# RishWijewardhena/vision-textile-inspection

Hardware: AMD Instinct MI355X
Metric: frames/sec whole-node, YOLOv8n-seg 640x640 bs=64; mask IoU vs CPU ref (higher is better)
Workload: dtype f16x2

## Files before the change

### vision-textile-inspection_amd/csrc/conv.hip

```cpp
#include <algorithm>
#include <cstdlib>
#include <type_traits>

#include "conv_dev.h"

namespace vti {

__host__ __device__ inline int patch_dim(int t, int ks, int s, int mode) { return mode == 1 ? t : (t - 1) * s + ks; }

size_t stem_lds_bytes(int TH, int TW);

bool conv_wreg_ok(int ks, int stride, int mode, int WN, int NREP, int threads) {
    return mode == 0 && ks == 1 && stride == 1 && threads == 256 && WN == 4 && NREP <= 4;
}

size_t conv_lds_bytes(int ks, int stride, int mode, int TH, int TW, int WN, int NREP, int wreg) {
    if (mode == 1) return stem_lds_bytes(TH, TW);
    const int npix = patch_dim(TH, ks, stride, mode) * patch_dim(TW, ks, stride, mode);
    const size_t plane = (size_t)((npix + 15) & ~15) * 16;
    const int taps = mode == 1 ? 1 : ks * ks;
    size_t raw = 0;
    if (mode == 1) raw = (((size_t)(2 * TH + 1) * (2 * TW + 1) * 3) + 15) & ~(size_t)15;
    return 4 * plane + (wreg ? 0 : (size_t)WN * NREP * taps * 1024) + raw;
}

template <typename T, int KS, int S, int NREP, int WN, int NREP2 = 0, int NT = 256, bool WREG = false>
__global__ __launch_bounds__(NT, NT == 512 ? 1 : 2) void conv_kernel(const ConvParams p) {
    using vec = typename Tr<T>::vec;
    constexpr int VEC = Tr<T>::VEC, KC = Tr<T>::KC;
    constexpr int TAPS = KS * KS, PAD = KS / 2;
    constexpr int NTB = WN * NREP;
    constexpr int PP = NT / 4;
    constexpr int AR = NT == 512 ? 6 : (S == 2 ? 12 : 8);
    constexpr int BR = (NTB * TAPS * 64 + NT - 1) / NT;
    static_assert(!WREG || (KS == 1 && WN == NT / 64 && NREP2 == 0 && BR == NREP && NREP < 5), "WREG: one consumer wave per fragment");
    constexpr unsigned OOB = 0xFFFFFFFFu;
    extern __shared__ __attribute__((aligned(16))) char smem[];

    const int tid = threadIdx.x, lane = tid & 63, wave = tid >> 6;
    const int wn = wave % WN, wm = wave / WN;
    int t = blockIdx.x;
    const int tx = t % p.tiles_x; t /= p.tiles_x;
    const int ty = t % p.tiles_y;
    const int b = t / p.tiles_y;
    const int oy0 = ty * p.TH, ox0 = tx * p.TW;
    const int PH = (p.TH - 1) * S + KS, PW = (p.TW - 1) * S + KS;
    const int npix = PH * PW;
    const int plane_bytes = ((npix + 15) & ~15) * 16;
    char* smA = smem;
    char* smB = smem + 4 * plane_bytes;
    const int nt0 = blockIdx.y * NTB;
    const int tile_px = p.TH * p.TW;
    VTI_STAMP(0);

    int abase[MREP], opy[MREP], opx[MREP];
    bool pvalid[MREP];
#pragma unroll
    for (int m = 0; m < MREP; ++m) {
        const int pp = (wm * MREP + m) * 16 + (lane & 15);
        const bool v = pp < tile_px;
        const int pc = v ? pp : 0;
        const int py = (int)__umulhi((unsigned)pc, p.tw_magic), px = pc - py * p.TW;
        opy[m] = oy0 + py; opx[m] = ox0 + px;
        pvalid[m] = v && opy[m] < p.Hout && opx[m] < p.Wout;
        abase[m] = (lane >> 4) * plane_bytes + ((py * S) * PW + px * S) * 16;
    }

    f32x4 acc[MREP][NREP];
#pragma unroll
    for (int m = 0; m < MREP; ++m)
#pragma unroll
        for (int n = 0; n < NREP; ++n) acc[m][n] = (f32x4){0.f, 0.f, 0.f, 0.f};

    const size_t frame_elems = (size_t)p.Hin * p.Win * p.in_ld;
    const __amdgpu_buffer_rsrc_t rsA = __builtin_amdgcn_make_buffer_rsrc(
        (void*)((const T*)p.in + (size_t)b * frame_elems), 0, (int)(frame_elems * sizeof(T)), 0x00020000);
    const __amdgpu_buffer_rsrc_t rsB = __builtin_amdgcn_make_buffer_rsrc((void*)p.wpk, 0, (int)p.wpk_bytes, 0x00020000);

    const int iy0 = oy0 * S - PAD, ix0 = ox0 * S - PAD;
    const int q = (tid >> 3) & 3;
    const int pix0 = (tid >> 5) * 8 + (tid & 7);
    const int ldsA0 = q * plane_bytes + pix0 * 16;
    const int cvalid = (p.Cin - q * VEC + KC - 1) / KC;
    unsigned aoff[AR];
#pragma unroll
    for (int u = 0; u < AR; ++u) {
        const int pix = pix0 + PP * u;
        const int py = (int)__umulhi((unsigned)pix, p.pw_magic), px = pix - py * PW;
        const int y = iy0 + py, x = ix0 + px;
        const bool ok = pix < npix && (unsigned)y < (unsigned)p.Hin && (unsigned)x < (unsigned)p.Win;
        aoff[u] = ok ? (unsigned)(((y * p.Win + x) * p.in_ld + p.in_coff + q * VEC) * (int)sizeof(T)) : OOB;
    }
    constexpr bool BPRE = NREP < 5 || NT == 512;
    constexpr int PD = (KS == 1 && BPRE) ? 2 : 1;
    vec ra[PD][AR], rb[PD][BR];
    auto loadB = [&](int c, vec (&rbs)[BR]) {
        const unsigned sB = (unsigned)(((size_t)c * p.ntiles_n + nt0) * (TAPS * 1024));
#pragma unroll
        for (int u = 0; u < BR; ++u) {
            if constexpr (WREG) rbs[u] = buf_load16<vec>(rsB, (unsigned)((wn * NREP + u) * 64 + lane) * 16u, sB);
            else if (tid + u * NT < NTB * TAPS * 64) rbs[u] = buf_load16<vec>(rsB, (unsigned)(tid + u * NT) * 16u, sB);
        }
    };
    auto issue = [&](int c, vec (&ras)[AR], vec (&rbs)[BR]) {
        const bool qok = c < cvalid;
#pragma unroll
        for (int u = 0; u < AR; ++u)
            if (pix0 + PP * u < ((npix + 7) & ~7))
                ras[u] = buf_load16<vec>(rsA, qok ? aoff[u] : OOB, (unsigned)(c * KC * (int)sizeof(T)));
        if constexpr (BPRE) loadB(c, rbs);
    };
    auto commit = [&](int c, vec (&ras)[AR], vec (&rbs)[BR]) {
        if constexpr (!BPRE) loadB(c, rbs);
#pragma unroll
        for (int u = 0; u < AR; ++u)
            if (pix0 + PP * u < npix) *(vec*)(smA + ldsA0 + u * (PP * 16)) = ras[u];
        if constexpr (!WREG) {
#pragma unroll
            for (int u = 0; u < BR; ++u)
                if (tid + u * NT < NTB * TAPS * 64) *(vec*)(smB + (tid + u * NT) * 16) = rbs[u];
        }
    };
    auto chunk = [&](int c, auto set_c) {
        constexpr int SET = decltype(set_c)::value;
        if (c < 2) VTI_STAMP(1 + 5 * c);
        commit(c, ra[SET], rb[SET]);
        if (c < 2) VTI_STAMP(3 + 5 * c);
        __syncthreads();
        if (c < 2) VTI_STAMP(4 + 5 * c);
        constexpr int WD = NREP >= 5 ? 1 : 2;
        vec wq[WD][NREP];
        if constexpr (WREG) {
#pragma unroll
            for (int n = 0; n < NREP; ++n) wq[0][n] = rb[SET][n];
        }
        if (c + PD < p.nchunks) issue(c + PD, ra[SET], rb[SET]);
        {
            constexpr int NSTEP = TAPS * MREP;
            constexpr int XD = NREP >= 5 ? 2 : 3;
            vec xq[XD];
            auto ldx = [&](int s_) -> vec {
                const int tp = s_ / MREP, mm = s_ % MREP;
                const int toff = ((tp / KS) * PW + (tp % KS)) * 16;
                return *(const vec*)(smA + abase[mm] + toff);
            };
            auto ldw = [&](int tp, vec (&w)[NREP]) {
#pragma unroll
                for (int n = 0; n < NREP; ++n)
                    w[n] = *(const vec*)(smB + ((wn * NREP + n) * TAPS + tp) * 1024 + lane * 16);
            };
            if constexpr (Tr<T>::H2 && TAPS > 1 && (NREP <= 3 || (NREP == 4 && NT == 512))) {
                auto ldw1 = [&](int tp, int n) -> vec { return *(const vec*)(smB + ((wn * NREP + n) * TAPS + tp) * 1024 + lane * 16); };
                h2_taps<NREP, MREP, TAPS, 3>(acc, ldx, ldw1);
            } else {
            if constexpr (!WREG) ldw(0, wq[0]);
            xq[0] = ldx(0);
            if (XD > 2 && NSTEP > 1) xq[1] = ldx(1);
#pragma unroll
            for (int s_ = 0; s_ < NSTEP; ++s_) {
                const int tp = s_ / MREP, mm = s_ % MREP;
                if (s_ + XD - 1 < NSTEP) xq[(s_ + XD - 1) % XD] = ldx(s_ + XD - 1);
                if (WD == 2 && mm == 0 && tp + 1 < TAPS) ldw(tp + 1, wq[(tp + 1) % WD]);
                __builtin_amdgcn_sched_barrier(0);
#pragma unroll
                for (int n = 0; n < NREP; ++n) acc[mm][n] = mma(wq[tp % WD][n], xq[s_ % XD], acc[mm][n]);
                __builtin_amdgcn_sched_barrier(0);
                if (WD == 1 && mm == MREP - 1 && tp + 1 < TAPS) ldw(tp + 1, wq[0]);
            }
            }
        }
        if (c < 2) VTI_STAMP(5 + 5 * c);
        if (c + 1 < p.nchunks) __syncthreads();
    };

    issue(0, ra[0], rb[0]);
    if constexpr (PD == 2) {
        if (p.nchunks > 1) issue(1, ra[1], rb[1]);
        for (int c = 0; c < p.nchunks; c += 2) {
            chunk(c, std::integral_constant<int, 0>{});
            if (c + 1 < p.nchunks) chunk(c + 1, std::integral_constant<int, 1>{});
        }
    } else {
        for (int c = 0; c < p.nchunks; ++c) chunk(c, std::integral_constant<int, 0>{});
    }

    VTI_STAMP(11);
    if constexpr (NREP2 == 0) {
        conv_epilogue<T, NREP>(p, acc, pvalid, opy, opx, b, nt0, wn, lane);
    } else {
        static_assert(WN == 1, "fused stage needs the whole Cout in one wave");
        conv_stage2<T, NREP, NREP2>(p, acc, pvalid, opy, opx, b, lane);
    }
    VTI_STAMP(12);
}

size_t convfold_lds_bytes(int TH, int TW) {
    const int npix = (TH + 2) * (TW + 2);
    return 4 * (size_t)((npix + 15) & ~15) * 16 + (size_t)16 * 4 * 1024;
}
bool convfold_supported(int c_in, int c_mid, int c_out, int ntiles2) {
    return c_in == c_mid && c_mid % 16 == 0 && c_out == 64 && c_in % 16 == 0 && c_in <= 64 && combo_has(FoldN2{}, ntiles2);
}

template <typename T, int NREP2, int NT = 256>
__global__ __launch_bounds__(NT, NT == 512 ? 1 : 2) void convfold_kernel(const ConvParams p) {
    using vec = typename Tr<T>::vec;
    constexpr int VEC = Tr<T>::VEC, KC = Tr<T>::KC;
    constexpr int NREP = 4, TAPS = 4, NTB = 16, AR = 8;
    constexpr int BR = NTB * TAPS * 64 / NT;
    constexpr int PPP = NT / 4;
    constexpr unsigned OOB = 0xFFFFFFFFu;
    extern __shared__ __attribute__((aligned(16))) char smem[];

    const int tid = threadIdx.x, lane = tid & 63, wave = (tid >> 6) & 3, mgrp = tid >> 8;
    const int py = wave >> 1, px = wave & 1;
    int t = blockIdx.x;
    const int tx = t % p.tiles_x; t /= p.tiles_x;
    const int ty = t % p.tiles_y;
    const int b = t / p.tiles_y;
    const int oy0 = ty * p.TH, ox0 = tx * p.TW;
    const int PH = p.TH + 2, PW = p.TW + 2;
    const int npix = PH * PW;
    const int plane_bytes = ((npix + 15) & ~15) * 16;
    char* smA = smem;
    char* smB = smem + 4 * plane_bytes;
    const int tile_px = p.TH * p.TW;

    int abase[MREP], opy[MREP], opx[MREP];
    bool pvalid[MREP];
#pragma unroll
    for (int m = 0; m < MREP; ++m) {
        const int pp = (mgrp * MREP + m) * 16 + (lane & 15);
        const bool v = pp < tile_px;
        const int pc = v ? pp : 0;
        const int ly = (int)__umulhi((unsigned)pc, p.tw_magic), lx = pc - ly * p.TW;
        pvalid[m] = v && oy0 + ly < p.Hout && ox0 + lx < p.Wout;
        opy[m] = 2 * (oy0 + ly) + py; opx[m] = 2 * (ox0 + lx) + px;
        abase[m] = (lane >> 4) * plane_bytes + ((ly + py) * PW + lx + px) * 16;
    }
    f32x4 acc[MREP][NREP];
#pragma unroll
    for (int m = 0; m < MREP; ++m)
#pragma unroll
        for (int n = 0; n < NREP; ++n) acc[m][n] = (f32x4){0.f, 0.f, 0.f, 0.f};

    const size_t frame_elems = (size_t)p.Hin * p.Win * p.in_ld;
    const __amdgpu_buffer_rsrc_t rsA = __builtin_amdgcn_make_buffer_rsrc(
        (void*)((const T*)p.in + (size_t)b * frame_elems), 0, (int)(frame_elems * sizeof(T)), 0x00020000);
    const __amdgpu_buffer_rsrc_t rsB = __builtin_amdgcn_make_buffer_rsrc((void*)p.wpk, 0, (int)p.wpk_bytes, 0x00020000);
    const int iy0 = oy0 - 1, ix0 = ox0 - 1;
    const int q = (tid >> 3) & 3;
    const int pix0 = (tid >> 5) * 8 + (tid & 7);
    const int ldsA0 = q * plane_bytes + pix0 * 16;
    const int cvalid = (p.Cin - q * VEC + KC - 1) / KC;
    unsigned aoff[AR];
#pragma unroll
    for (int u = 0; u < AR; ++u) {
        const int pix = pix0 + PPP * u;
        const int ry = (int)__umulhi((unsigned)pix, p.pw_magic), rx = pix - ry * PW;
        const int y = iy0 + ry, x = ix0 + rx;
        const bool ok = pix < npix && (unsigned)y < (unsigned)p.Hin && (unsigned)x < (unsigned)p.Win;
        aoff[u] = ok ? (unsigned)(((y * p.Win + x) * p.in_ld + p.in_coff + q * VEC) * (int)sizeof(T)) : OOB;
    }
    vec ra[AR];
    auto issue = [&](int c) {
        const bool qok = c < cvalid;
#pragma unroll
        for (int u = 0; u < AR; ++u)
            if (pix0 + PPP * u < ((npix + 7) & ~7))
                ra[u] = buf_load16<vec>(rsA, qok ? aoff[u] : OOB, (unsigned)(c * KC * (int)sizeof(T)));
    };
    auto commit = [&](int c) {
        const unsigned sB = (unsigned)((size_t)c * (NTB * TAPS * 1024));
#pragma unroll
        for (int h = 0; h < 2; ++h) {
            vec rb[BR / 2];
#pragma unroll
            for (int u = 0; u < BR / 2; ++u) rb[u] = buf_load16<vec>(rsB, (unsigned)(tid + (h * (BR / 2) + u) * NT) * 16u, sB);
            if (h == 0) {
#pragma unroll
                for (int u = 0; u < AR; ++u)
                    if (pix0 + PPP * u < npix) *(vec*)(smA + ldsA0 + u * (PPP * 16)) = ra[u];
            }
#pragma unroll
            for (int u = 0; u < BR / 2; ++u) *(vec*)(smB + (tid + (h * (BR / 2) + u) * NT) * 16) = rb[u];
        }
    };

    issue(0);
    for (int c = 0; c < p.nchunks; ++c) {
        commit(c);
        __syncthreads();
        if (c + 1 < p.nchunks) issue(c + 1);
        {
            constexpr int NSTEP = TAPS * MREP;
            vec xq[3];
            vec wq[2][NREP];
            auto ldx = [&](int s_) -> vec {
                const int tp = s_ / MREP, mm = s_ % MREP;
                return *(const vec*)(smA + abase[mm] + ((tp >> 1) * PW + (tp & 1)) * 16);
            };
            auto ldw = [&](int tp, vec (&w)[NREP]) {
#pragma unroll
                for (int n = 0; n < NREP; ++n) w[n] = *(const vec*)(smB + ((wave * NREP + n) * TAPS + tp) * 1024 + lane * 16);
            };
            if constexpr (Tr<T>::H2) {
                auto ldw1 = [&](int tp, int n) -> vec { return *(const vec*)(smB + ((wave * NREP + n) * TAPS + tp) * 1024 + lane * 16); };
                h2_taps<NREP, MREP, TAPS, 3>(acc, ldx, ldw1);
            } else {
            ldw(0, wq[0]);
            xq[0] = ldx(0);
            xq[1] = ldx(1);
#pragma unroll
            for (int s_ = 0; s_ < NSTEP; ++s_) {
                const int tp = s_ / MREP, mm = s_ % MREP;
                if (s_ + 2 < NSTEP) xq[(s_ + 2) % 3] = ldx(s_ + 2);
                if (mm == 0 && tp + 1 < TAPS) ldw(tp + 1, wq[(tp + 1) % 2]);
                __builtin_amdgcn_sched_barrier(0);
#pragma unroll
                for (int n = 0; n < NREP; ++n) acc[mm][n] = mma(wq[tp % 2][n], xq[s_ % 3], acc[mm][n]);
                __builtin_amdgcn_sched_barrier(0);
            }
            }
        }
        if (c + 1 < p.nchunks) __syncthreads();
    }
    conv_stage2<T, NREP, NREP2, true>(p, acc, pvalid, opy, opx, b, lane);
}

hipError_t launch_convfold(int dtype, const ConvParams& p, size_t lds_bytes, hipStream_t st) {
    dim3 grid((unsigned)(p.B * p.tiles_y * p.tiles_x));
    if (grid.x == 0) return hipSuccess;
    const int nthr = p.nt == 512 ? 512 : 256;
    if (p.TH * p.TW > (nthr / 256) * MREP * 16 || ((p.TH + 2) * (p.TW + 2) + 7) / 8 * 32 > nthr * 8 || p.Cout != 256 || !p.out2 || !p.fold)
        return hipErrorInvalidValue;
    return with_conv_type(dtype, [&](auto t) -> hipError_t {
        using T = typename decltype(t)::type;
        if (p.nt == 512) {
            if constexpr (sizeof(T) == 4)
                return combo_dispatch(FoldN2{}, [&](auto c) {
                    return launch_lds<convfold_kernel<T, decltype(c)::v[0], 512>>(grid, dim3(512), lds_bytes, st, p);
                }, p.ntiles2);
            return hipErrorInvalidValue;
        }
        return combo_dispatch(FoldN2{}, [&](auto c) {
            return launch_lds<convfold_kernel<T, decltype(c)::v[0]>>(grid, dim3(256), lds_bytes, st, p);
        }, p.ntiles2);
    });
}

template <typename T, int NREP>
__global__ __launch_bounds__(256) void stem_kernel(const ConvParams p) {
    using vec = typename Tr<T>::vec;
    constexpr int VEC = Tr<T>::VEC, KC = Tr<T>::KC;
    constexpr int NCH = 32 / KC;
    extern __shared__ __attribute__((aligned(16))) char smem[];
    T* lut = (T*)smem;
    unsigned* raw32 = (unsigned*)(smem + 1024);
    const unsigned char* raw = (const unsigned char*)raw32;

    const int tid = threadIdx.x, lane = tid & 63, wave = tid >> 6;
    int t = blockIdx.x;
    const int tx = t % p.tiles_x; t /= p.tiles_x;
    const int ty = t % p.tiles_y;
    const int b = t / p.tiles_y;
    const int oy0 = ty * p.TH, ox0 = tx * p.TW;
    const int RH = 2 * p.TH + 1, RWB = (2 * p.TW + 1) * 3;
    const int RWD = (RWB + 6) >> 2;
    const int pitch = RWD * 4;
    const int x0b = (ox0 * 2 - 1) * 3, a0 = x0b & ~3, shift = x0b - a0;
    const int y0 = oy0 * 2 - 1;
    const uint8_t* inb = (const uint8_t*)p.in + (size_t)b * p.Hin * p.Win * 3;
    const int rowbytes = p.Win * 3;
    if ((rowbytes & 3) == 0 && RH * RWD <= 8 * 256) {
        unsigned vv[8];
#pragma unroll
        for (int it = 0; it < 8; ++it) {
            const int i = tid + it * 256;
            const int ry = (int)__umulhi((unsigned)i, p.rw_magic), rd = i - ry * RWD;
            const int y = y0 + ry, gx = a0 + 4 * rd;
            const bool ok = i < RH * RWD && (unsigned)y < (unsigned)p.Hin && gx >= 0 && gx < rowbytes;
            vv[it] = *(const unsigned*)(inb + (ok ? (size_t)y * rowbytes + gx : (size_t)0));
        }
#pragma unroll
        for (int it = 0; it < 8; ++it) {
            const int i = tid + it * 256;
            const int ry = (int)__umulhi((unsigned)i, p.rw_magic), rd = i - ry * RWD;
            const int y = y0 + ry, gx = a0 + 4 * rd;
            const bool ok = (unsigned)y < (unsigned)p.Hin && gx >= 0 && gx < rowbytes;
            if (i < RH * RWD) raw32[i] = ok ? vv[it] : 0u;
        }
    } else
    for (int i = tid; i < RH * RWD; i += 256) {
        const int ry = (int)__umulhi((unsigned)i, p.rw_magic), rd = i - ry * RWD;
        const int y = y0 + ry, gx = a0 + 4 * rd;
        unsigned v = 0;
        if ((unsigned)y < (unsigned)p.Hin) {
            if ((rowbytes & 3) == 0) {
                if (gx >= 0 && gx < rowbytes) v = *(const unsigned*)(inb + (size_t)y * rowbytes + gx);
            } else {
#pragma unroll
                for (int k = 0; k < 4; ++k)
                    if (gx + k >= 0 && gx + k < rowbytes) v |= (unsigned)inb[(size_t)y * rowbytes + gx + k] << (8 * k);
            }
        }
        raw32[i] = v;
    }
    lut[tid] = to_T<T>((float)tid / 255.0f);
    __syncthreads();

    const int tile_px = p.TH * p.TW;
    const int nt0 = blockIdx.y * NREP;
    int opy[MREP], opx[MREP], rbase[MREP];
    bool pvalid[MREP];
#pragma unroll
    for (int m = 0; m < MREP; ++m) {
        const int pp = (wave * MREP + m) * 16 + (lane & 15);
        const bool v = pp < tile_px;
        const int pc = v ? pp : 0;
        const int py = (int)__umulhi((unsigned)pc, p.tw_magic), px = pc - py * p.TW;
        opy[m] = oy0 + py; opx[m] = ox0 + px;
        pvalid[m] = v && opy[m] < p.Hout && opx[m] < p.Wout;
        rbase[m] = (py * 2) * pitch + (px * 2) * 3 + shift;
    }
    f32x4 acc[MREP][NREP];
#pragma unroll
    for (int m = 0; m < MREP; ++m)
#pragma unroll
        for (int n = 0; n < NREP; ++n) acc[m][n] = (f32x4){0.f, 0.f, 0.f, 0.f};
#pragma unroll
    for (int c = 0; c < NCH; ++c) {
        int off[VEC];
#pragma unroll
        for (int j = 0; j < VEC; ++j) {
            const int k = c * KC + (lane >> 4) * VEC + j;
            const int tap = k / 3, chn = k - tap * 3;
            const int kh = tap / 3, kw = tap - kh * 3;
            off[j] = k < 27 ? kh * pitch + kw * 3 + (p.swap_rb ? 2 - chn : chn) : -1;
        }
        vec w[NREP];
#pragma unroll
        for (int n = 0; n < NREP; ++n) {
            const int nt = nt0 + n < p.ntiles_n ? nt0 + n : 0;
            w[n] = ((const vec*)p.wpk)[((size_t)c * p.ntiles_n + nt) * 64 + lane];
        }
#pragma unroll
        for (int m = 0; m < MREP; ++m) {
            vec x;
#pragma unroll
            for (int j = 0; j < VEC; ++j) vset<T>(x, j, off[j] >= 0 ? lut[raw[rbase[m] + off[j]]] : to_T<T>(0.f));
#pragma unroll
            for (int n = 0; n < NREP; ++n) acc[m][n] = mma(w[n], x, acc[m][n]);
        }
    }
    conv_epilogue<T, NREP>(p, acc, pvalid, opy, opx, b, nt0, 0, lane);
}

constexpr int SL_TH = 8, SL_TW = 40;
constexpr int SL_SH = 2 * SL_TH + 1, SL_SW = 2 * SL_TW + 1, SL_NSP = SL_SH * SL_SW;
constexpr int SL_RH = 4 * SL_TH + 3, SL_RWB = (4 * SL_TW + 3) * 3, SL_RWD = (SL_RWB + 6) >> 2;
constexpr int sl_pitch(int es) { return es == 2 ? 520 : 512; }
constexpr int SL_NJ = (SL_SW + 3) / 4, SL_NWIN = SL_SH * SL_NJ;
static_assert(24 * (SL_NJ - 1) + 32 <= 512 && SL_RWD * 4 <= 512, "stem windows must stay inside a patch row");

size_t stem_l1_lds_bytes(int dtype) {
    const size_t es = dtype == VTI_F16 ? 2 : 4, pes = dtype == VTI_F32 ? 4 : 2;
    return (((size_t)SL_RH * sl_pitch((int)pes) * pes + 15) & ~(size_t)15) + (size_t)SL_NSP * 16 * es;
}

template <typename T>
__global__ __launch_bounds__(256, sizeof(T) == 2 ? 2 : 1) void stem_l1_kernel(const ConvParams p) {
    using vec = typename Tr<T>::vec;
    constexpr int ES = (int)sizeof(T);
    constexpr bool XH = Tr<T>::H2;
    using PT = typename std::conditional<XH, half_t, T>::type;
    using pvec = typename Tr<PT>::vec;
    constexpr int VEC = Tr<PT>::VEC, KC = Tr<PT>::KC, PES = (int)sizeof(PT);
    constexpr int NCH = 32 / KC;
    constexpr int NWP = XH ? 2 : 1;
    constexpr int NS1 = sizeof(T) == 2 ? 5 : 9;
    constexpr bool FAST = !Tr<T>::F32;
    constexpr int SL_PITCH = sl_pitch(PES);
    constexpr int CP_BYTES = (SL_RH * SL_PITCH * PES + 15) & ~15;
    extern __shared__ __attribute__((aligned(16))) char smem[];
    PT* cp = (PT*)smem;
    char* sout = smem + CP_BYTES;

    const int tid = threadIdx.x, lane = tid & 63, wave = tid >> 6, g = lane >> 4;
    const int ntiles = p.B * p.tiles_y * p.tiles_x;
    if ((int)blockIdx.x >= ntiles) return;
    const int Hs = (p.Hin - 1) / 2 + 1, Ws = (p.Win - 1) / 2 + 1;
    const int rowbytes = p.Win * 3;
    auto tile_geom = [&](int tt, int& b_, int& oy0_, int& ox0_) {
        const int tx = tt % p.tiles_x, r = tt / p.tiles_x;
        b_ = r / p.tiles_y; oy0_ = (r % p.tiles_y) * SL_TH; ox0_ = tx * SL_TW;
    };
    VTI_STAMP(0);
    constexpr int RC = (SL_RWD + 63) / 64, NR = (SL_RH + 3) / 4;
    unsigned vv[NR][RC];
    const bool aligned = (rowbytes & 3) == 0;
    auto issue_raw = [&](int tt) {
        int b_, oy0_, ox0_;
        tile_geom(tt, b_, oy0_, ox0_);
        const int iy0_ = 2 * (2 * oy0_ - 1) - 1, a0_ = ((2 * (2 * ox0_ - 1) - 1) * 3) & ~3;
        const uint8_t* inb_ = (const uint8_t*)p.in + (size_t)b_ * p.Hin * p.Win * 3;
#pragma unroll
        for (int it = 0; it < NR; ++it) {
            const int ry = wave + 4 * it;
            const int y = iy0_ + ry;
            const bool row_ok = ry < SL_RH && (unsigned)y < (unsigned)p.Hin;
#pragma unroll
            for (int ch = 0; ch < RC; ++ch) {
                const int rd = lane + 64 * ch;
                const int gx = a0_ + 4 * rd;
                const bool ok = row_ok && rd < SL_RWD && gx >= 0 && gx < rowbytes;
                vv[it][ch] = *(const unsigned*)(inb_ + (ok ? (size_t)y * rowbytes + gx : (size_t)0));
            }
        }
    };
    if (aligned) issue_raw((int)blockIdx.x);
    for (int t = (int)blockIdx.x; t < ntiles; t += (int)gridDim.x) {
    int b, oy0, ox0;
    tile_geom(t, b, oy0, ox0);
    const int sy0 = 2 * oy0 - 1, sx0 = 2 * ox0 - 1;
    const int iy0 = 2 * sy0 - 1;
    const int x0b = (2 * sx0 - 1) * 3, a0 = x0b & ~3;
    const uint8_t* inb = (const uint8_t*)p.in + (size_t)b * p.Hin * p.Win * 3;
    const void* w0p = p.w0;
    const void* w1p = p.wpk;
    asm volatile("" : "+s"(w0p), "+s"(w1p));
    pvec wA[4][3][NCH * NWP];
    {
        const pvec* w0 = (const pvec*)w0p + (size_t)(p.swap_rb ? 1 : 0) * (4 * 3 * NCH * NWP * 64);
#pragma unroll
        for (int pp = 0; pp < 4; ++pp)
#pragma unroll
            for (int kh = 0; kh < 3; ++kh)
#pragma unroll
                for (int c = 0; c < NCH * NWP; ++c) wA[pp][kh][c] = w0[(size_t)((pp * 3 + kh) * NCH * NWP + c) * 64 + lane];
    }
    vec w1all[NS1][2];
#pragma unroll
    for (int s1 = 0; s1 < NS1; ++s1)
#pragma unroll
        for (int n = 0; n < 2; ++n) w1all[s1][n] = ((const vec*)w1p)[((size_t)s1 * 2 + n) * 64 + lane];
    const f32x4 bias0_4 = *(const f32x4*)(p.bias0 + g * 4);
    Stage2Regs<T, 2, 2> s2r;
    if (p.out2) stage2_preload<T, 2, 2>(p, lane, false, s2r);
    {
        if (aligned) {
#pragma unroll
            for (int it = 0; it < NR; ++it) {
                const int ry = wave + 4 * it;
                const int y = iy0 + ry;
                const bool row_ok = ry < SL_RH && (unsigned)y < (unsigned)p.Hin;
#pragma unroll
                for (int ch = 0; ch < RC; ++ch) {
                    const int rd = lane + 64 * ch;
                    const int gx = a0 + 4 * rd;
                    const bool ok = row_ok && rd < SL_RWD && gx >= 0 && gx < rowbytes;
                    vv[it][ch] = ok ? vv[it][ch] : 0u;
                }
            }
        } else {
#pragma unroll
            for (int it = 0; it < NR; ++it) {
                const int ry = wave + 4 * it;
                const int y = iy0 + ry;
                const bool row_ok = ry < SL_RH && (unsigned)y < (unsigned)p.Hin;
#pragma unroll
                for (int ch = 0; ch < RC; ++ch) {
                    const int rd = lane + 64 * ch;
                    const int gx = a0 + 4 * rd;
                    unsigned v = 0;
                    if (row_ok && rd < SL_RWD) {
#pragma unroll
                        for (int k = 0; k < 4; ++k)
                            if (gx + k >= 0 && gx + k < rowbytes) v |= (unsigned)inb[(size_t)y * rowbytes + gx + k] << (8 * k);
                    }
                    vv[it][ch] = v;
                }
            }
        }
#pragma unroll
        for (int it = 0; it < NR; ++it) {
            const int ry = wave + 4 * it;
#pragma unroll
            for (int ch = 0; ch < RC; ++ch) {
                const int rd = lane + 64 * ch;
                if (ry >= SL_RH || rd >= SL_RWD) continue;
                const unsigned v = vv[it][ch];
                PT* o = cp + (size_t)ry * SL_PITCH + 4 * rd;
                if constexpr (XH) {
                    half4 hv;
#pragma unroll
                    for (int k = 0; k < 4; ++k) hv[k] = (half_t)(float)((v >> (8 * k)) & 0xffu);
                    *(half4*)o = hv;
                } else if constexpr (sizeof(T) == 2) {
                    half4 hv;
#pragma unroll
                    for (int k = 0; k < 4; ++k) hv[k] = (half_t)((float)((v >> (8 * k)) & 0xffu) * (1.0f / 255.0f));
                    *(half4*)o = hv;
                } else {
#pragma unroll
                    for (int k = 0; k < 4; ++k) o[k] = to_T<T>((float)((v >> (8 * k)) & 0xffu) / 255.0f);
                }
            }
        }
    }
    for (int i = tid; i < SL_RH * ((SL_PITCH - 4 * SL_RWD) / 4); i += 256) {
        const int ry = i / ((SL_PITCH - 4 * SL_RWD) / 4), c4 = i - ry * ((SL_PITCH - 4 * SL_RWD) / 4);
        PT* o = cp + (size_t)ry * SL_PITCH + 4 * SL_RWD + 4 * c4;
        o[0] = to_T<PT>(0.f); o[1] = to_T<PT>(0.f); o[2] = to_T<PT>(0.f); o[3] = to_T<PT>(0.f);
    }
    __syncthreads();
    VTI_STAMP(1);
    if (aligned && t + (int)gridDim.x < ntiles) issue_raw(t + (int)gridDim.x);
    {
        const f32x4 bias4 = bias0_4;
        constexpr int NBLK = (SL_NWIN + 15) / 16;
        for (int blk = wave; blk < NBLK; blk += 4) {
            const int wi = blk * 16 + (lane & 15);
            const bool wvalid = wi < SL_NWIN;
            const int wc = wvalid ? wi : SL_NWIN - 1;
            const int J = wc / SL_SH, sy = wc - J * SL_SH;
            const PT* base = cp + (size_t)(2 * sy) * SL_PITCH + 24 * J + g * VEC;
            pvec x[3][NCH];
#pragma unroll
            for (int kh = 0; kh < 3; ++kh)
#pragma unroll
                for (int c = 0; c < NCH; ++c) x[kh][c] = *(const pvec*)(base + kh * SL_PITCH + c * KC);
            f32x4 acc[4];
#pragma unroll
            for (int pp = 0; pp < 4; ++pp) {
                acc[pp] = (f32x4){0.f, 0.f, 0.f, 0.f};
#pragma unroll
                for (int kh = 0; kh < 3; ++kh)
#pragma unroll
                    for (int c = 0; c < NCH; ++c)
#pragma unroll
                        for (int wp = 0; wp < NWP; ++wp) acc[pp] = mma(wA[pp][kh][c * NWP + wp], x[kh][c], acc[pp]);
            }
            const bool row_in = (unsigned)(sy0 + sy) < (unsigned)Hs;
#pragma unroll
            for (int pp = 0; pp < 4; ++pp) {
                const int sx = 4 * J + pp;
                f32x4 v = silu4<FAST>(acc_bias<T>(acc[pp], bias4, p.alpha0));
                if (!(row_in && (unsigned)(sx0 + sx) < (unsigned)Ws)) v = (f32x4){0.f, 0.f, 0.f, 0.f};
                if (wvalid && sx < SL_SW) {
                    T* o = (T*)(sout + ((size_t)(sy * SL_SW + sx) * 16 + g * 4) * ES);
                    if constexpr (sizeof(T) == 2) {
                        half4 hv;
#pragma unroll
                        for (int j = 0; j < 4; ++j) hv[j] = (half_t)v[j];
                        *(half4*)o = hv;
                    } else {
                        *(u32x4*)o = pack4<T>(v);
                    }
                }
            }
        }
    }
    __syncthreads();
    VTI_STAMP(2);
    int opy[MREP], opx[MREP], sbase[MREP];
    bool pvalid[MREP];
#pragma unroll
    for (int m = 0; m < MREP; ++m) {
        const int pp = (wave * MREP + m) * 16 + (lane & 15);
        const int py = pp / SL_TW, px = pp - py * SL_TW;
        opy[m] = oy0 + py; opx[m] = ox0 + px;
        pvalid[m] = opy[m] < p.Hout && opx[m] < p.Wout;
        sbase[m] = ((2 * py) * SL_SW + 2 * px) * 16 * ES;
    }
    f32x4 acc[MREP][2];
#pragma unroll
    for (int m = 0; m < MREP; ++m) { acc[m][0] = (f32x4){0.f, 0.f, 0.f, 0.f}; acc[m][1] = (f32x4){0.f, 0.f, 0.f, 0.f}; }
#pragma unroll
    for (int s = 0; s < NS1; ++s) {
        const int tap = sizeof(T) == 2 ? 2 * s + (g >> 1) : s;
        const int tc = tap < 9 ? tap : 8;
        const int toff = ((tc / 3) * SL_SW + (tc % 3)) * 16 * ES + (sizeof(T) == 2 ? (g & 1) * 8 : g * 4) * ES;
        vec w1[2];
#pragma unroll
        for (int n = 0; n < 2; ++n) w1[n] = w1all[s][n];
#pragma unroll
        for (int m = 0; m < MREP; ++m) {
            const vec x = *(const vec*)(sout + sbase[m] + toff);
#pragma unroll
            for (int n = 0; n < 2; ++n) acc[m][n] = mma(w1[n], x, acc[m][n]);
        }
    }
    VTI_STAMP(3);
    if (p.out2) conv_stage2<T, 2, 2, false, true>(p, acc, pvalid, opy, opx, b, lane, &s2r);
    else conv_epilogue<T, 2>(p, acc, pvalid, opy, opx, b, 0, 0, lane);
    VTI_STAMP(12);
    }
}

void stem_l1_tile(int* th, int* tw) { *th = SL_TH; *tw = SL_TW; }

int stem_l1_grid(int dtype, int ntiles, bool persistent) {
    const int wgpc = (int)std::min<size_t>(2, (160 * 1024) / stem_l1_lds_bytes(dtype));
    if (!persistent) return ntiles;
    return std::min(ntiles, 256 * std::max(1, wgpc));
}

hipError_t launch_stem_l1(int dtype, const ConvParams& p, hipStream_t st, bool persistent) {
    dim3 grid((unsigned)stem_l1_grid(dtype, p.B * p.tiles_y * p.tiles_x, persistent));
    if (grid.x == 0) return hipSuccess;
    const size_t lds = stem_l1_lds_bytes(dtype);
    return with_conv_type(dtype, [&](auto t) { return launch_lds<stem_l1_kernel<typename decltype(t)::type>>(grid, dim3(256), lds, st, p); });
}

size_t stem_lds_bytes(int TH, int TW) { return 1024 + (size_t)(2 * TH + 1) * ((((2 * TW + 1) * 3 + 6) >> 2) * 4); }

using ConvTile3 = Combos<Ints<1, 1>, Ints<2, 1>, Ints<3, 1>, Ints<4, 1>, Ints<5, 1>, Ints<1, 2>, Ints<2, 2>, Ints<1, 4>>;
using ConvTile1 = decltype(concat(ConvTile3{}, Combos<Ints<3, 2>, Ints<4, 2>, Ints<5, 2>, Ints<2, 4>, Ints<3, 4>, Ints<4, 4>, Ints<5, 4>>{}));
using ConvTile1W = Combos<Ints<1, 4>, Ints<2, 4>, Ints<3, 4>, Ints<4, 4>>;
using StemNrep = Combos<Ints<1>, Ints<2>, Ints<3>, Ints<4>, Ints<5>>;

bool conv_cfg_fits(int ks, int stride, int mode, int TH, int TW, int WN, int NREP, int threads) {
    if (mode == 1) return WN == 1 && (2 * TH + 1) * (((2 * TW + 1) * 3 + 6) >> 2) < 65536;
    if (threads != 256 && !(threads == 512 && ks == 3 && stride == 1 && WN == 1)) return false;
    const int AR = threads == 512 ? 6 : (stride == 2 ? 12 : 8);
    const int npix = patch_dim(TH, ks, stride, mode) * patch_dim(TW, ks, stride, mode);
    if (((npix + 7) / 8) * 32 > threads * AR) return false;
    return ks == 1 ? combo_has(ConvTile1{}, NREP, WN) : combo_has(ConvTile3{}, NREP, WN);
}

bool conv_fusable(int nrep, int nrep2) { return combo_has(FusedPairs{}, nrep, nrep2); }

template <typename T, int KS, int S>
static hipError_t launch_ks(int nrep, const ConvParams& p, dim3 grid, size_t lds, hipStream_t st) {
    if constexpr (KS == 1) {
        if (p.wreg)
            return combo_dispatch(ConvTile1W{}, [&](auto c) {
                return launch_lds<conv_kernel<T, 1, 1, decltype(c)::v[0], 4, 0, 256, true>>(grid, dim3(256), lds, st, p);
            }, nrep, p.WN);
    }
    return combo_dispatch(std::conditional_t<KS == 1, ConvTile1, ConvTile3>{}, [&](auto c) {
        using C = decltype(c);
        return launch_lds<conv_kernel<T, KS, S, C::v[0], C::v[1]>>(grid, dim3(256), lds, st, p);
    }, nrep, p.WN);
}

template <typename T>
static hipError_t launch_t(int ks, int stride, int nrep, int mode, const ConvParams& p, dim3 grid, size_t lds,
                           hipStream_t st) {
    if (p.ntiles2 > 0) {
        if (!(ks == 3 && stride == 1 && p.WN == 1 && mode == 0)) return hipErrorInvalidValue;
        return combo_dispatch(FusedPairs{}, [&](auto c) {
            using C = decltype(c);
            return p.nt == 512 ? launch_lds<conv_kernel<T, 3, 1, C::v[0], 1, C::v[1], 512>>(grid, dim3(512), lds, st, p)
                               : launch_lds<conv_kernel<T, 3, 1, C::v[0], 1, C::v[1]>>(grid, dim3(256), lds, st, p);
        }, nrep, p.ntiles2);
    }
    if (mode == 1)
        return combo_dispatch(StemNrep{}, [&](auto c) {
            hipLaunchKernelGGL((stem_kernel<T, decltype(c)::v[0]>), grid, dim3(256), lds, st, p);
            return hipGetLastError();
        }, nrep);
    if (ks == 1 && stride == 1) return launch_ks<T, 1, 1>(nrep, p, grid, lds, st);
    if (ks == 3 && stride == 1) return launch_ks<T, 3, 1>(nrep, p, grid, lds, st);
    if (ks == 3 && stride == 2) return launch_ks<T, 3, 2>(nrep, p, grid, lds, st);
    return hipErrorInvalidValue;
}

hipError_t launch_conv(int dtype, int ks, int stride, int nrep, int mode, const ConvParams& p, size_t lds_bytes,
                       hipStream_t st) {
    if (p.pk == 4) return launch_conv_pk2(dtype, nrep, p, lds_bytes, st);
    if (p.pk == 3) return launch_bneck_pk(dtype, nrep, p, lds_bytes, st);
    if (p.pk == 2) return launch_conv1_pk(dtype, nrep, p, lds_bytes, st);
    if (p.pk) return launch_conv_pk(dtype, nrep, p, lds_bytes, st);
    const int NTB = p.WN * nrep;
    dim3 grid((unsigned)(p.B * p.tiles_y * p.tiles_x), (unsigned)((p.ntiles_n + NTB - 1) / NTB));
    if (grid.x == 0) return hipSuccess;
    const int nwaves = p.nt == 512 ? 8 : 4;
    if (p.wreg && !conv_wreg_ok(ks, stride, mode, p.WN, nrep, p.nt)) return hipErrorInvalidValue;
    lds_bytes = std::max(lds_bytes, conv_lds_bytes(ks, stride, mode, p.TH, p.TW, p.WN, nrep, p.wreg));
    if ((p.nt != 256 && p.nt != 512) || (p.nt == 512 && p.ntiles2 == 0)) return hipErrorInvalidValue;
    if (p.TH * p.TW > (nwaves / p.WN) * MREP * 16 || (p.WN != 1 && p.WN != 2 && p.WN != 4)) return hipErrorInvalidValue;
    return with_conv_type(dtype, [&](auto t) { return launch_t<typename decltype(t)::type>(ks, stride, nrep, mode, p, grid, lds_bytes, st); });
}

}
```

### vision-textile-inspection_amd/csrc/misc.hip

```cpp
#include "vti_internal.h"

namespace vti {

typedef _Float16 half_t;
typedef _Float16 half8 __attribute__((ext_vector_type(8)));
typedef float f32x4 __attribute__((ext_vector_type(4)));

typedef unsigned u32x4 __attribute__((ext_vector_type(4)));
struct h2e { unsigned u; };
__device__ __forceinline__ float h2_val(unsigned u) {
    return (float)__builtin_bit_cast(half_t, (unsigned short)(u & 0xffffu)) + (float)__builtin_bit_cast(half_t, (unsigned short)(u >> 16));
}

template <typename T> struct V16;
template <> struct V16<half_t> { typedef half8 vec; static constexpr int N = 8; };
template <> struct V16<float> { typedef f32x4 vec; static constexpr int N = 4; };
template <> struct V16<h2e> { typedef u32x4 vec; static constexpr int N = 4; };

__device__ __forceinline__ half8 vmax(half8 a, half8 b) { return __builtin_elementwise_max(a, b); }
__device__ __forceinline__ f32x4 vmax(f32x4 a, f32x4 b) { return __builtin_elementwise_max(a, b); }
__device__ __forceinline__ u32x4 vmax(u32x4 a, u32x4 b) {
    u32x4 r;
#pragma unroll
    for (int j = 0; j < 4; ++j) r[j] = h2_val(b[j]) > h2_val(a[j]) ? b[j] : a[j];
    return r;
}
template <typename T> __device__ __forceinline__ typename V16<T>::vec vlowest() {
    typename V16<T>::vec v;
    if constexpr (sizeof(T) == 4 && !__is_same(T, float)) {
#pragma unroll
        for (int j = 0; j < 4; ++j) v[j] = 0xfc00u;
    } else {
#pragma unroll
        for (int j = 0; j < V16<T>::N; ++j) v[j] = (T)(-INFINITY);
    }
    return v;
}

template <typename T>
__global__ __launch_bounds__(256) void sppf_pool_kernel(const PoolParams p) {
    using vec = typename V16<T>::vec;
    constexpr int N = V16<T>::N;
    const int cv = p.C / N;
    const long total = (long)p.B * p.H * p.W * cv;
    for (long i = blockIdx.x * 256L + threadIdx.x; i < total; i += (long)gridDim.x * 256) {
        const int c = (int)(i % cv);
        long r = i / cv;
        const int x = (int)(r % p.W); r /= p.W;
        const int y = (int)(r % p.H);
        const int b = (int)(r / p.H);
        const T* in = (const T*)p.in;
        vec m5 = vlowest<T>(), m9 = vlowest<T>(), m13 = vlowest<T>();
        for (int dy = -6; dy <= 6; ++dy) {
            const int yy = y + dy;
            if ((unsigned)yy >= (unsigned)p.H) continue;
            for (int dx = -6; dx <= 6; ++dx) {
                const int xx = x + dx;
                if ((unsigned)xx >= (unsigned)p.W) continue;
                const vec v = *(const vec*)(in + ((size_t)(b * p.H + yy) * p.W + xx) * p.ld + p.in_coff + c * N);
                const int ad = max(abs(dy), abs(dx));
                m13 = vmax(m13, v);
                if (ad <= 4) m9 = vmax(m9, v);
                if (ad <= 2) m5 = vmax(m5, v);
            }
        }
        T* o = (T*)p.out + ((size_t)(b * p.H + y) * p.W + x) * p.ld + p.out_coff + c * N;
        *(vec*)o = m5;
        *(vec*)(o + p.C) = m9;
        *(vec*)(o + 2 * p.C) = m13;
    }
}

template <typename T, int G>
__global__ __launch_bounds__(256) void sppf_pool_lds_kernel(const PoolParams p) {
    using vec = typename V16<T>::vec;
    constexpr int N = V16<T>::N;
    extern __shared__ __attribute__((aligned(16))) char smem[];
    const int HW = p.H * p.W;
    vec* cur = (vec*)smem;
    vec* tmp = cur + HW * G;
    const int cg = p.C / (N * G);
    const int b = blockIdx.x / cg, c = blockIdx.x - b * cg;
    const T* in = (const T*)p.in + (size_t)b * HW * p.ld + p.in_coff + c * (N * G);
    T* out = (T*)p.out + (size_t)b * HW * p.ld + p.out_coff + c * (N * G);
    {
        constexpr int MAXIT = 8;
        if (HW * G <= MAXIT * 256) {
            vec r[MAXIT];
#pragma unroll
            for (int it = 0; it < MAXIT; ++it) {
                const int i = threadIdx.x + it * 256;
                const int ic = i < HW * G ? i : 0;
                r[it] = *(const vec*)(in + (size_t)(ic / G) * p.ld + (ic % G) * N);
            }
#pragma unroll
            for (int it = 0; it < MAXIT; ++it) {
                const int i = threadIdx.x + it * 256;
                if (i < HW * G) cur[i] = r[it];
            }
        } else {
            for (int i = threadIdx.x; i < HW * G; i += 256) cur[i] = *(const vec*)(in + (size_t)(i / G) * p.ld + (i % G) * N);
        }
    }
    __syncthreads();
    for (int pass = 0; pass < 3; ++pass) {
        for (int i = threadIdx.x; i < HW * G; i += 256) {
            const int pix = i / G, v_ = i - pix * G;
            const int y = pix / p.W, x = pix - y * p.W;
            vec m = cur[i];
            for (int d = -2; d <= 2; ++d) {
                const int xx = x + d;
                if (d == 0 || (unsigned)xx >= (unsigned)p.W) continue;
                const vec v = cur[(y * p.W + xx) * G + v_];
                m = vmax(m, v);
            }
            tmp[i] = m;
        }
        __syncthreads();
        for (int i = threadIdx.x; i < HW * G; i += 256) {
            const int pix = i / G, v_ = i - pix * G;
            const int y = pix / p.W, x = pix - y * p.W;
            vec m = tmp[i];
            for (int d = -2; d <= 2; ++d) {
                const int yy = y + d;
                if (d == 0 || (unsigned)yy >= (unsigned)p.H) continue;
                const vec v = tmp[(yy * p.W + x) * G + v_];
                m = vmax(m, v);
            }
            cur[i] = m;
            *(vec*)(out + (size_t)pix * p.ld + pass * p.C + v_ * N) = m;
        }
        __syncthreads();
    }
}

hipError_t launch_sppf_pool(int dtype, const PoolParams& p, hipStream_t st) {
    const int N = dtype == VTI_F16 ? 8 : 4;
    const long total = (long)p.B * p.H * p.W * (p.C / N);
    if (total == 0) return hipSuccess;
    const size_t lds1 = (size_t)2 * p.H * p.W * 16;
    if (lds1 * 4 <= 64 * 1024 && p.C % (4 * N) == 0) {
        const int grid = p.B * (p.C / (4 * N));
        if (dtype == VTI_F16) hipLaunchKernelGGL((sppf_pool_lds_kernel<half_t, 4>), dim3(grid), dim3(256), lds1 * 4, st, p);
        else if (dtype == VTI_H2) hipLaunchKernelGGL((sppf_pool_lds_kernel<h2e, 4>), dim3(grid), dim3(256), lds1 * 4, st, p);
        else hipLaunchKernelGGL((sppf_pool_lds_kernel<float, 4>), dim3(grid), dim3(256), lds1 * 4, st, p);
        return hipGetLastError();
    }
    if (lds1 <= 64 * 1024) {
        const int grid = p.B * (p.C / N);
        if (dtype == VTI_F16) hipLaunchKernelGGL((sppf_pool_lds_kernel<half_t, 1>), dim3(grid), dim3(256), lds1, st, p);
        else if (dtype == VTI_H2) hipLaunchKernelGGL((sppf_pool_lds_kernel<h2e, 1>), dim3(grid), dim3(256), lds1, st, p);
        else hipLaunchKernelGGL((sppf_pool_lds_kernel<float, 1>), dim3(grid), dim3(256), lds1, st, p);
        return hipGetLastError();
    }
    const int grid = (int)((total + 255) / 256 < 4096 ? (total + 255) / 256 : 4096);
    if (dtype == VTI_F16) hipLaunchKernelGGL(sppf_pool_kernel<half_t>, dim3(grid), dim3(256), 0, st, p);
    else if (dtype == VTI_H2) hipLaunchKernelGGL(sppf_pool_kernel<h2e>, dim3(grid), dim3(256), 0, st, p);
    else hipLaunchKernelGGL(sppf_pool_kernel<float>, dim3(grid), dim3(256), 0, st, p);
    return hipGetLastError();
}

template <typename T>
__global__ __launch_bounds__(256) void upsample2x_kernel(const Up2Params p) {
    using vec = typename V16<T>::vec;
    constexpr int N = V16<T>::N;
    const int cv = p.C / N;
    const int Ho = 2 * p.H, Wo = 2 * p.W;
    const long total = (long)p.B * Ho * Wo * cv;
    for (long i = blockIdx.x * 256L + threadIdx.x; i < total; i += (long)gridDim.x * 256) {
        const int c = (int)(i % cv);
        long r = i / cv;
        const int x = (int)(r % Wo); r /= Wo;
        const int y = (int)(r % Ho);
        const int b = (int)(r / Ho);
        const vec v = *(const vec*)((const T*)p.in + ((size_t)(b * p.H + (y >> 1)) * p.W + (x >> 1)) * p.in_ld + p.in_coff + c * N);
        *(vec*)((T*)p.out + ((size_t)(b * Ho + y) * Wo + x) * p.out_ld + p.out_coff + c * N) = v;
    }
}

hipError_t launch_upsample2x(int dtype, const Up2Params& p, hipStream_t st) {
    const long total = (long)p.B * 4 * p.H * p.W * (p.C / (dtype == VTI_F16 ? 8 : 4));
    if (total == 0) return hipSuccess;
    const int grid = (int)((total + 255) / 256 < 4096 ? (total + 255) / 256 : 4096);
    if (dtype == VTI_F16) hipLaunchKernelGGL(upsample2x_kernel<half_t>, dim3(grid), dim3(256), 0, st, p);
    else hipLaunchKernelGGL(upsample2x_kernel<float>, dim3(grid), dim3(256), 0, st, p);
    return hipGetLastError();
}

constexpr int DEC_TA = 64;

__global__ __launch_bounds__(256) void decode_kernel(const DecodeParams p, int tiles0, int tiles1, int tiles_per_frame) {
    extern __shared__ __attribute__((aligned(16))) float tile[];
    const int b = blockIdx.x / tiles_per_frame;
    int t = blockIdx.x - b * tiles_per_frame;
    int l = 0;
    if (t >= tiles0 + tiles1) { l = 2; t -= tiles0 + tiles1; } else if (t >= tiles0) { l = 1; t -= tiles0; }
    const int W = p.W[l], HW = p.H[l] * W;
    const int la0 = t * DEC_TA;
    const int na = min(DEC_TA, HW - la0);
    const int nbox = 4 * p.reg_max, nin = nbox + p.nc + p.nm, pitch = nin + 1;
    const int tid = threadIdx.x;
    const size_t pix0 = (size_t)b * HW + la0;
    const float* src = p.box[l] + pix0 * nbox;
    for (int i = tid; i < na * nbox; i += 256) { const int a = i / nbox, k = i - a * nbox; tile[a * pitch + k] = src[i]; }
    src = p.cls[l] + pix0 * p.nc;
    for (int i = tid; i < na * p.nc; i += 256) { const int a = i / p.nc, k = i - a * p.nc; tile[a * pitch + nbox + k] = src[i]; }
    src = p.mc[l] + pix0 * p.nm;
    for (int i = tid; i < na * p.nm; i += 256) { const int a = i / p.nm, k = i - a * p.nm; tile[a * pitch + nbox + p.nc + k] = src[i]; }
    __syncthreads();
    float dist = 0.f;
    const int a_ = tid >> 2, side = tid & 3;
    if (a_ < na) {
        const float* v = tile + a_ * pitch + side * 16;
        float e[16];
        float mx = -INFINITY;
#pragma unroll
        for (int k = 0; k < 16; ++k) { e[k] = v[k]; mx = fmaxf(mx, e[k]); }
        float sum = 0.f;
#pragma unroll
        for (int k = 0; k < 16; ++k) { e[k] = expf(e[k] - mx); sum += e[k]; }
#pragma unroll
        for (int k = 0; k < 16; ++k) dist += (e[k] / sum) * (float)k;
    }
    __syncthreads();
    if (a_ < na) tile[a_ * pitch + side] = dist;
    __syncthreads();
    const int no = 4 + p.nc + p.nm;
    float* out = p.pred + ((size_t)b * p.A + p.a0[l] + la0) * no;
    const float st = (float)p.stride[l];
    for (int i = tid; i < no * DEC_TA; i += 256) {
        const int a = i / no, ch = i - a * no;
        if (a >= na) continue;
        const float* r = tile + a * pitch;
        float v;
        if (ch < 4) {
            const int la = la0 + a;
            const int gy = la / W, gx = la - gy * W;
            const float ax = (float)gx + 0.5f, ay = (float)gy + 0.5f;
            const float x1 = ax - r[0], y1 = ay - r[1], x2 = ax + r[2], y2 = ay + r[3];
            v = ch == 0 ? ((x1 + x2) / 2.0f) * st : ch == 1 ? ((y1 + y2) / 2.0f) * st : ch == 2 ? (x2 - x1) * st : (y2 - y1) * st;
        } else if (ch < 4 + p.nc) {
            v = 1.0f / (1.0f + expf(-r[nbox + ch - 4]));
        } else {
            v = r[nbox + ch - 4];
        }
        out[(size_t)a * no + ch] = v;
    }
}

hipError_t launch_decode(const DecodeParams& p, hipStream_t st) {
    if ((long)p.B * p.A == 0) return hipSuccess;
    if (p.reg_max != 16) return hipErrorInvalidValue;
    int tiles[3];
    for (int l = 0; l < 3; ++l) tiles[l] = (p.H[l] * p.W[l] + DEC_TA - 1) / DEC_TA;
    const int tpf = tiles[0] + tiles[1] + tiles[2];
    const size_t lds = (size_t)DEC_TA * (4 * p.reg_max + p.nc + p.nm + 1) * sizeof(float);
    if (lds > 64 * 1024) return hipErrorInvalidValue;
    hipLaunchKernelGGL(decode_kernel, dim3((unsigned)(p.B * tpf)), dim3(256), lds, st, p, tiles[0], tiles[1], tpf);
    return hipGetLastError();
}

__global__ __launch_bounds__(256) void box_decode_kernel(const DecodeParams p, int tiles0, int tiles1, int tiles_per_frame) {
    __shared__ float tile[DEC_TA * 65];
    __shared__ float dist4[DEC_TA * 4];
    const int b = blockIdx.x / tiles_per_frame;
    int t = blockIdx.x - b * tiles_per_frame;
    int l = 0;
    if (t >= tiles0 + tiles1) { l = 2; t -= tiles0 + tiles1; } else if (t >= tiles0) { l = 1; t -= tiles0; }
    const int W = p.W[l], HW = p.H[l] * W;
    const int la0 = t * DEC_TA;
    const int na = min(DEC_TA, HW - la0);
    const int tid = threadIdx.x;
    const float* src = p.box[l] + ((size_t)b * HW + la0) * 64;
    for (int i = tid; i < na * 64; i += 256) tile[(i >> 6) * 65 + (i & 63)] = src[i];
    __syncthreads();
    const int a_ = tid >> 2, side = tid & 3;
    if (a_ < na) {
        const float* v = tile + a_ * 65 + side * 16;
        float e[16];
        float mx = -INFINITY;
#pragma unroll
        for (int k = 0; k < 16; ++k) { e[k] = v[k]; mx = fmaxf(mx, e[k]); }
        float sum = 0.f, dist = 0.f;
#pragma unroll
        for (int k = 0; k < 16; ++k) { e[k] = expf(e[k] - mx); sum += e[k]; }
#pragma unroll
        for (int k = 0; k < 16; ++k) dist += (e[k] / sum) * (float)k;
        dist4[a_ * 4 + side] = dist;
    }
    __syncthreads();
    const int no = 4 + p.nc + p.nm;
    const float st = (float)p.stride[l];
    const int a = tid >> 2, ch = tid & 3;
    if (a < na) {
        const float* r = dist4 + a * 4;
        const int la = la0 + a;
        const int gy = la / W, gx = la - gy * W;
        const float ax = (float)gx + 0.5f, ay = (float)gy + 0.5f;
        const float x1 = ax - r[0], y1 = ay - r[1], x2 = ax + r[2], y2 = ay + r[3];
        const float v = ch == 0 ? ((x1 + x2) / 2.0f) * st : ch == 1 ? ((y1 + y2) / 2.0f) * st : ch == 2 ? (x2 - x1) * st : (y2 - y1) * st;
        p.pred[((size_t)b * p.A + p.a0[l] + la) * no + ch] = v;
    }
}

hipError_t launch_box_decode(const DecodeParams& p, hipStream_t st) {
    if ((long)p.B * p.A == 0) return hipSuccess;
    if (p.reg_max != 16) return hipErrorInvalidValue;
    int tiles[3];
    for (int l = 0; l < 3; ++l) tiles[l] = (p.H[l] * p.W[l] + DEC_TA - 1) / DEC_TA;
    const int tpf = tiles[0] + tiles[1] + tiles[2];
    hipLaunchKernelGGL(box_decode_kernel, dim3((unsigned)(p.B * tpf)), dim3(256), 0, st, p, tiles[0], tiles[1], tpf);
    return hipGetLastError();
}

template <typename T>
__global__ void debug_nchw_kernel(const T* src, int B, int H, int W, int C, int ld, int coff, float* dst) {
    const long total = (long)B * C * H * W;
    for (long i = blockIdx.x * 256L + threadIdx.x; i < total; i += (long)gridDim.x * 256) {
        const int x = (int)(i % W);
        long r = i / W;
        const int y = (int)(r % H); r /= H;
        const int c = (int)(r % C);
        const int b = (int)(r / C);
        if constexpr (sizeof(T) == 4 && !__is_same(T, float)) dst[i] = h2_val(src[((size_t)(b * H + y) * W + x) * ld + coff + c].u) * (1.0f / 16.0f);
        else dst[i] = (float)src[((size_t)(b * H + y) * W + x) * ld + coff + c];
    }
}

hipError_t launch_debug_nchw(int elem_is_f32, const void* src, int B, int H, int W, int C, int ld, int coff,
                             float* dst, hipStream_t st) {
    const long total = (long)B * C * H * W;
    if (total == 0) return hipSuccess;
    const int grid = (int)((total + 255) / 256 < 8192 ? (total + 255) / 256 : 8192);
    if (elem_is_f32 == 2) hipLaunchKernelGGL(debug_nchw_kernel<h2e>, dim3(grid), dim3(256), 0, st, (const h2e*)src, B, H, W, C, ld, coff, dst);
    else if (elem_is_f32) hipLaunchKernelGGL(debug_nchw_kernel<float>, dim3(grid), dim3(256), 0, st, (const float*)src, B, H, W, C, ld, coff, dst);
    else hipLaunchKernelGGL(debug_nchw_kernel<half_t>, dim3(grid), dim3(256), 0, st, (const half_t*)src, B, H, W, C, ld, coff, dst);
    return hipGetLastError();
}

}
```

Measured before the change: 16030.

## Swizzle stem LDS layout for 32-bit types and use order-preserving keys for h2 pooling

After: 15840. 0.988x the previous value.

```diff
diff --git a/vision-textile-inspection_amd/csrc/conv.hip b/vision-textile-inspection_amd/csrc/conv.hip
--- a/vision-textile-inspection_amd/csrc/conv.hip
+++ b/vision-textile-inspection_amd/csrc/conv.hip
@@ -466,6 +466,11 @@
 size_t stem_l1_lds_bytes(int dtype) {
     const size_t es = dtype == VTI_F16 ? 2 : 4, pes = dtype == VTI_F32 ? 4 : 2;
     return (((size_t)SL_RH * sl_pitch((int)pes) * pes + 15) & ~(size_t)15) + (size_t)SL_NSP * 16 * es;
+}
+
+template <int ES> __device__ __forceinline__ int sl_unit(int g, int sx, int sy) {
+    if constexpr (ES == 4) return g ^ ((sx >> 2) & 3) ^ (sy & 2);
+    else return g;
 }
 
 template <typename T>
@@ -642,13 +647,14 @@
                         for (int wp = 0; wp < NWP; ++wp) acc[pp] = mma(wA[pp][kh][c * NWP + wp], x[kh][c], acc[pp]);
             }
             const bool row_in = (unsigned)(sy0 + sy) < (unsigned)Hs;
+            const int un = sl_unit<ES>(g, 4 * J, sy);
 #pragma unroll
             for (int pp = 0; pp < 4; ++pp) {
                 const int sx = 4 * J + pp;
                 f32x4 v = silu4<FAST>(acc_bias<T>(acc[pp], bias4, p.alpha0));
                 if (!(row_in && (unsigned)(sx0 + sx) < (unsigned)Ws)) v = (f32x4){0.f, 0.f, 0.f, 0.f};
                 if (wvalid && sx < SL_SW) {
-                    T* o = (T*)(sout + ((size_t)(sy * SL_SW + sx) * 16 + g * 4) * ES);
+                    T* o = (T*)(sout + ((size_t)(sy * SL_SW + sx) * 16 + un * 4) * ES);
                     if constexpr (sizeof(T) == 2) {
                         half4 hv;
 #pragma unroll
@@ -665,6 +671,8 @@
     VTI_STAMP(2);
     int opy[MREP], opx[MREP], sbase[MREP];
     bool pvalid[MREP];
+    static_assert(SL_TW % 4 == 0, "swz: px & 3 must not depend on the m-tile");
+    [[maybe_unused]] const int swz = (lane & 1) * (16 + ((lane & 2) << 4));
 #pragma unroll
     for (int m = 0; m < MREP; ++m) {
         const int pp = (wave * MREP + m) * 16 + (lane & 15);
@@ -672,6 +680,9 @@
         opy[m] = oy0 + py; opx[m] = ox0 + px;
         pvalid[m] = opy[m] < p.Hout && opx[m] < p.Wout;
         sbase[m] = ((2 * py) * SL_SW + 2 * px) * 16 * ES;
+        if constexpr (ES == 4) {
+            sbase[m] += sl_unit<ES>(g, 2 * px, 2 * py) * 16;
+        }
     }
     f32x4 acc[MREP][2];
 #pragma unroll
@@ -680,13 +691,19 @@
     for (int s = 0; s < NS1; ++s) {
         const int tap = sizeof(T) == 2 ? 2 * s + (g >> 1) : s;
         const int tc = tap < 9 ? tap : 8;
-        const int toff = ((tc / 3) * SL_SW + (tc % 3)) * 16 * ES + (sizeof(T) == 2 ? (g & 1) * 8 : g * 4) * ES;
+        const int toff = ((tc / 3) * SL_SW + (tc % 3)) * 16 * ES + (sizeof(T) == 2 ? (g & 1) * 8 * ES : 0);
         vec w1[2];
 #pragma unroll
         for (int n = 0; n < 2; ++n) w1[n] = w1all[s][n];
 #pragma unroll
         for (int m = 0; m < MREP; ++m) {
-            const vec x = *(const vec*)(sout + sbase[m] + toff);
+            int sb = sbase[m];
+            if constexpr (ES == 4) {
+                if (s % 3 == 2) sb ^= swz;
+                if (s / 3 == 2) sb ^= 2 * 16;
+                if (s % 3 == 2 || s / 3 == 2) asm volatile("" : "+v"(sb));
+            }
+            const vec x = *(const vec*)(sout + sb + toff);
 #pragma unroll
             for (int n = 0; n < 2; ++n) acc[m][n] = mma(w1[n], x, acc[m][n]);
         }
diff --git a/vision-textile-inspection_amd/csrc/misc.hip b/vision-textile-inspection_amd/csrc/misc.hip
--- a/vision-textile-inspection_amd/csrc/misc.hip
+++ b/vision-textile-inspection_amd/csrc/misc.hip
@@ -11,6 +11,18 @@
 __device__ __forceinline__ float h2_val(unsigned u) {
     return (float)__builtin_bit_cast(half_t, (unsigned short)(u & 0xffffu)) + (float)__builtin_bit_cast(half_t, (unsigned short)(u >> 16));
 }
+typedef unsigned short u16x2 __attribute__((ext_vector_type(2)));
+typedef short s16x2 __attribute__((ext_vector_type(2)));
+__device__ __forceinline__ u16x2 h2_flip(u16x2 x, u16x2 m) { return (x ^ m) + ((m & (unsigned short)0x8001) ^ (unsigned short)0x8000); }
+__device__ __forceinline__ unsigned h2_to_key(unsigned u) {
+    const u16x2 x = __builtin_bit_cast(u16x2, u);
+    const unsigned k = __builtin_bit_cast(unsigned, h2_flip(x, __builtin_bit_cast(u16x2, __builtin_bit_cast(s16x2, x) >> 15)));
+    return (k << 16) | (k >> 16);
+}
+__device__ __forceinline__ unsigned h2_from_key(unsigned key) {
+    const u16x2 k = __builtin_bit_cast(u16x2, (key << 16) | (key >> 16));
+    return __builtin_bit_cast(unsigned, h2_flip(k, __builtin_bit_cast(u16x2, __builtin_bit_cast(s16x2, ~k) >> 15)));
+}
 
 template <typename T> struct V16;
 template <> struct V16<half_t> { typedef half8 vec; static constexpr int N = 8; };
@@ -19,17 +31,26 @@
 
 __device__ __forceinline__ half8 vmax(half8 a, half8 b) { return __builtin_elementwise_max(a, b); }
 __device__ __forceinline__ f32x4 vmax(f32x4 a, f32x4 b) { return __builtin_elementwise_max(a, b); }
-__device__ __forceinline__ u32x4 vmax(u32x4 a, u32x4 b) {
-    u32x4 r;
-#pragma unroll
-    for (int j = 0; j < 4; ++j) r[j] = h2_val(b[j]) > h2_val(a[j]) ? b[j] : a[j];
-    return r;
+__device__ __forceinline__ u32x4 vmax(u32x4 a, u32x4 b) { return __builtin_elementwise_max(a, b); }
+template <typename T> __device__ __forceinline__ typename V16<T>::vec pool_in(typename V16<T>::vec v) {
+    if constexpr (__is_same(T, h2e)) {
+#pragma unroll
+        for (int j = 0; j < 4; ++j) v[j] = h2_to_key(v[j]);
+    }
+    return v;
+}
+template <typename T> __device__ __forceinline__ typename V16<T>::vec pool_out(typename V16<T>::vec v) {
+    if constexpr (__is_same(T, h2e)) {
+#pragma unroll
+        for (int j = 0; j < 4; ++j) v[j] = h2_from_key(v[j]);
+    }
+    return v;
 }
 template <typename T> __device__ __forceinline__ typename V16<T>::vec vlowest() {
     typename V16<T>::vec v;
-    if constexpr (sizeof(T) == 4 && !__is_same(T, float)) {
-#pragma unroll
-        for (int j = 0; j < 4; ++j) v[j] = 0xfc00u;
+    if constexpr (__is_same(T, h2e)) {
+#pragma unroll
+        for (int j = 0; j < 4; ++j) v[j] = 0x04008000u;
     } else {
 #pragma unroll
         for (int j = 0; j < V16<T>::N; ++j) v[j] = (T)(-INFINITY);
@@ -57,7 +78,7 @@
             for (int dx = -6; dx <= 6; ++dx) {
                 const int xx = x + dx;
                 if ((unsigned)xx >= (unsigned)p.W) continue;
-                const vec v = *(const vec*)(in + ((size_t)(b * p.H + yy) * p.W + xx) * p.ld + p.in_coff + c * N);
+                const vec v = pool_in<T>(*(const vec*)(in + ((size_t)(b * p.H + yy) * p.W + xx) * p.ld + p.in_coff + c * N));
                 const int ad = max(abs(dy), abs(dx));
                 m13 = vmax(m13, v);
                 if (ad <= 4) m9 = vmax(m9, v);
@@ -65,9 +86,9 @@
             }
         }
         T* o = (T*)p.out + ((size_t)(b * p.H + y) * p.W + x) * p.ld + p.out_coff + c * N;
-        *(vec*)o = m5;
-        *(vec*)(o + p.C) = m9;
-        *(vec*)(o + 2 * p.C) = m13;
+        *(vec*)o = pool_out<T>(m5);
+        *(vec*)(o + p.C) = pool_out<T>(m9);
+        *(vec*)(o + 2 * p.C) = pool_out<T>(m13);
     }
 }
 
@@ -96,10 +117,10 @@
 #pragma unroll
             for (int it = 0; it < MAXIT; ++it) {
                 const int i = threadIdx.x + it * 256;
-                if (i < HW * G) cur[i] = r[it];
+                if (i < HW * G) cur[i] = pool_in<T>(r[it]);
             }
         } else {
-            for (int i = threadIdx.x; i < HW * G; i += 256) cur[i] = *(const vec*)(in + (size_t)(i / G) * p.ld + (i % G) * N);
+            for (int i = threadIdx.x; i < HW * G; i += 256) cur[i] = pool_in<T>(*(const vec*)(in + (size_t)(i / G) * p.ld + (i % G) * N));
         }
     }
     __syncthreads();
@@ -128,7 +149,7 @@
                 m = vmax(m, v);
             }
             cur[i] = m;
-            *(vec*)(out + (size_t)pix * p.ld + pass * p.C + v_ * N) = m;
+            *(vec*)(out + (size_t)pix * p.ld + pass * p.C + v_ * N) = pool_out<T>(m);
         }
         __syncthreads();
     }
```
